# ActiveIntelligentSystemsLab/moving_object_detector

Hardware: AMD Instinct MI355X
Metric: stereo pairs/sec (scene-flow+cluster) at 1280x720 (higher is better)
Workload: dtype f32+f64; 1 GPU; 1280x720 synthetic sequence (zed-style camera), scene-flow + cluster kernels only (disparity/flow precomputed, HBM-resident), reference default parameters; distinct_frames_per_gpu=16, outputs=six cloud planes, dynamic mask, objects, cluster-label plane, batch_chunks=0, stream=one synthetic stream, contiguous chunk per rank + one disparity plane of halo, collective_executed=True, collective_backend=nccl, collective_on_device=True, collective_world_size=1

## Files before the change

moving_object_detector_amd/csrc/cluster_final.hip:

```cpp
#include "cluster_common.h"
#include <algorithm>
#pragma clang fp contract(off)
namespace {

#ifndef FINAL_PLAIN_LABELS
#define FINAL_ST(p, v) __builtin_nontemporal_store((int)(v), (p))
#else
#define FINAL_ST(p, v) (*(p) = (v))
#endif
constexpr int kFinalEarly = 32;
template <int TH, int NW, bool XY_FROM_Z>
__global__ __launch_bounds__(NW * 64) void k_final(DevCam c, ClArgs a) {
  constexpr int RPW = TH / NW;
  __shared__ int nlmap[TH * 64];
  __shared__ int lcount[TH * 64];
  const int wi = blockIdx.x, f = blockIdx.z, lane = threadIdx.x, w = __builtin_amdgcn_readfirstlane((int)threadIdx.y);
  const size_t tidx = (size_t)f * gridDim.y * gridDim.x + (size_t)blockIdx.y * gridDim.x + wi;
  const size_t N = (size_t)c.W * c.H;
  const size_t fN = (size_t)f * N;
  const int x0 = wi * 64, y0 = blockIdx.y * TH, r0 = w * RPW, x = x0 + lane;
  if (a.tilehdr[tidx * 2] == 0) {
    if (a.labels) {
#pragma unroll
      for (int j = 0; j < RPW; j++) { const int y = y0 + r0 + j; if (y < c.H && x < c.W) FINAL_ST(&a.labels[fN + (size_t)y * c.W + x], -1); }
    }
    return;
  }
  const int xc = min(x, c.W - 1);
  uint64_t mw[RPW], rw[RPW];
  int par[RPW];
#pragma unroll
  for (int j = 0; j < RPW; j++) {
    const int y = y0 + r0 + j, yc = min(y, c.H - 1);
    const size_t wo = ((size_t)f * c.H + yc) * c.mask_words + wi;
    mw[j] = (y < c.H) ? a.mask[wo] : 0ull;
    rw[j] = (y < c.H) ? a.lroot[wo] : 0ull;
    par[j] = a.parent[fN + (size_t)yc * c.W + xc];
  }
#pragma unroll
  for (int j = 0; j < RPW; j++) {
    if ((rw[j] >> lane) & 1ull) {
      const int cell = (r0 + j) * 64 + lane;
      const int p = (y0 + r0 + j) * c.W + x;
      int lab = -1, first = 0;
      if (MOD_CHECK(a, par[j] >= 0 && (size_t)par[j] < N, 5)) {
        const int fr = par[j];
        lab = a.rkey[fN + fr];
        const int seg = a.rsize[fN + fr];
        const int own = a.rkey[fN + p];
        first = seg + (fr == p ? 0 : own);
      }
      nlmap[cell] = lab;
      lcount[cell] = first;
    }
  }
  float vx[RPW], vy[RPW], vz[RPW], px[RPW], py[RPW], pz[RPW];
  int ndyn = 0;
#pragma unroll
  for (int j = 0; j < RPW; j++) ndyn += __popcll((unsigned long long)mw[j]);
  const bool early = ndyn >= kFinalEarly;
  auto load_members = [&]() {
#pragma unroll
    for (int j = 0; j < RPW; j++) {
      const size_t gp = fN + (size_t)min(y0 + r0 + j, c.H - 1) * c.W + xc;
      vx[j] = a.vx[gp]; vy[j] = a.vy[gp]; vz[j] = a.vz[gp];
      pz[j] = a.z[gp];
      if (!XY_FROM_Z) { px[j] = a.x[gp]; py[j] = a.y[gp]; }
    }
  };
  if (early) load_members();
  lds_barrier();
  if (w == 0 && lane == 0) a.tilehdr[tidx * 2] = 0;
  const float invW = 1.0f / (float)c.W;
  const int tile0 = y0 * c.W + x0;
  int nl[RPW], cell[RPW], slot[RPW];
  bool any_member = false;
#pragma unroll
  for (int j = 0; j < RPW; j++) {
    const int y = y0 + r0 + j;
    const bool dyn = (mw[j] >> lane) & 1ull;
    const int d = par[j] - tile0;
    const int ly = (int)(((float)d + 0.5f) * invW);
    const bool isroot = (rw[j] >> lane) & 1ull;
    int cl = !dyn ? 0 : isroot ? ((r0 + j) * 64 + lane) : (ly * 64 + (d - ly * c.W));
    if (!MOD_CHECK(a, cl >= 0 && cl < TH * 64 && (!dyn || isroot || (d >= 0 && d - ly * c.W < 64)), 6)) cl = 0;
    int l = dyn ? nlmap[cl] : -1;
    if (!MOD_CHECK(a, l >= -1 && l < a.max_objects, 7)) l = -1;
    nl[j] = l; cell[j] = cl; slot[j] = 0;
    if (a.labels && y < c.H && x < c.W) FINAL_ST(&a.labels[fN + (size_t)y * c.W + x], l);
    any_member = any_member || (__ballot(l >= 0) != 0);
  }
  if (any_member) {
    if (!early) load_members();
#pragma unroll
    for (int j = 0; j < RPW; j++) {
      const int l = nl[j], cl = cell[j];
      const uint64_t mb = __ballot(l >= 0);
      if (mb == 0) continue;
      const int lead = __ffsll((unsigned long long)mb) - 1;
      const int c0 = __builtin_amdgcn_readlane(cl, lead);
      const bool grp = l >= 0 && cl == c0;
      const uint64_t gb = __ballot(grp);
      int base = 0;
      if (lane == lead) base = atomicAdd(&lcount[c0], __popcll((unsigned long long)gb));
      base = __builtin_amdgcn_readlane(base, lead);
      if (grp) slot[j] = base + __popcll((unsigned long long)(gb & ((1ull << lane) - 1ull)));
      else if (l >= 0) slot[j] = atomicAdd(&lcount[cl], 1);
    }
    if (XY_FROM_Z) {
      const double rx = c.rayx[xc];
#pragma unroll
      for (int j = 0; j < RPW; j++) {
        const double zd = (double)pz[j];
        px[j] = (float)(rx * zd);
        py[j] = (float)(c.rayy[min(y0 + r0 + j, c.H - 1)] * zd);
      }
    }
    uint32_t nb[RPW];
#pragma unroll
    for (int j = 0; j < RPW; j++) nb[j] = __float_as_uint(norm3_f32(vx[j], vy[j], vz[j]));
#pragma unroll
    for (int j = 0; j < RPW; j++) {
      if (nl[j] >= 0) {
        if (MOD_CHECK(a, slot[j] >= 0 && (size_t)slot[j] < N, 8)) {
          a.mbits[fN + slot[j]] = nb[j];
          a.mpix[fN + slot[j]] = (uint32_t)((y0 + r0 + j) * c.W + x);
        }
      }
    }
    int pend[RPW];
#pragma unroll
    for (int j = 0; j < RPW; j++) pend[j] = nl[j];
    for (;;) {
      int mine = -1;
#pragma unroll
      for (int j = 0; j < RPW; j++) mine = pend[j] >= 0 ? pend[j] : mine;
      const uint64_t b = __ballot(mine >= 0);
      if (b == 0) break;
      const int L = __builtin_amdgcn_readlane(mine, __ffsll((unsigned long long)b) - 1);
      uint32_t mn0 = 0xffffffffu, mn1 = 0xffffffffu, mn2 = 0xffffffffu, mx0 = 0u, mx1 = 0u, mx2 = 0u, mn3 = 0xffffffffu, mx3 = 0u;
#pragma unroll
      for (int j = 0; j < RPW; j++) {
        if (pend[j] == L) {
          const uint32_t ox = f2ord(px[j]), oy = f2ord(py[j]), oz = f2ord(pz[j]);
          mn0 = min(mn0, ox); mx0 = max(mx0, ox); mn1 = min(mn1, oy); mx1 = max(mx1, oy); mn2 = min(mn2, oz); mx2 = max(mx2, oz);
          mn3 = min(mn3, nb[j]); mx3 = max(mx3, nb[j]);
          pend[j] = -1;
        }
      }
      mn0 = wave_min_u32(mn0); mn1 = wave_min_u32(mn1); mn2 = wave_min_u32(mn2); mn3 = wave_min_u32(mn3);
      mx0 = wave_max_u32(mx0); mx1 = wave_max_u32(mx1); mx2 = wave_max_u32(mx2); mx3 = wave_max_u32(mx3);
      uint32_t v = ~mx3;
      v = lane == 0 ? mn0 : v; v = lane == 1 ? mn1 : v; v = lane == 2 ? mn2 : v; v = lane == 3 ? ~mx0 : v; v = lane == 4 ? ~mx1 : v;
// ... 44 lines not shown
  uint32_t *cstart = reinterpret_cast<uint32_t *>(&lraw[kMemCells]);
  __shared__ int s_box[4], s_sum[kMemThreads / 64 + 1];
  for (int f = blockIdx.x; f < frames; f += gridDim.x) {
    const ClusterInfo *C = a.clusters + (size_t)f * a.max_objects;
    const int K = min(a.counters[f * kClusterCounters + 1], a.max_objects);
    const int total = K > 0 ? C[K - 1].offset + C[K - 1].size : 0;
    int32_t *o = m.offsets + (size_t)f * (a.max_objects + 1);
    for (int k = tid; k <= a.max_objects; k += kMemThreads) o[k] = k < K ? C[k].offset : total;
  }
  auto segment = [&](uint32_t item, int &size, int &off) {
    const ClusterInfo *ci = a.clusters + item;
    size = ci->size; off = ci->offset;
    return size >= 1 && off >= 0 && (size_t)off + (size_t)size <= N;
  };
  for (int wi = blockIdx.x; wi < nwork; wi += gridDim.x) {
    const uint32_t item = a.worklist[wi];
    int size, off;
    if (!segment(item, size, off) || size <= kMemWaveMax) continue;
    members_of<kMemThreads, kMemCells, XY_FROM_Z, POINTS>(c, a, m, item, size, off, cmask, cstart, s_box, s_sum, tid);
  }
  __syncthreads();
  for (int wi = blockIdx.x * (kMemThreads / 64) + wv; wi < nwork; wi += gridDim.x * (kMemThreads / 64)) {
    const uint32_t item = a.worklist[wi];
    int size, off;
    if (!segment(item, size, off) || size > kMemWaveMax) continue;
    members_of<64, kMemWaveCells, XY_FROM_Z, POINTS>(c, a, m, item, size, off, cmask + wv * kMemWaveCells, cstart + wv * kMemWaveCells, nullptr,
                                                     nullptr, lane);
  }
}
}

void launch_final(const DevCam &c, const ClArgs &a, int frames, hipStream_t s) {
  constexpr int kFinalWaves = 2;
  if (a.xy_from_z) hipLaunchKernelGGL((k_final<kTileH, kFinalWaves, true>), tile_grid(c, frames), dim3(64, kFinalWaves, 1), 0, s, c, a);
  else hipLaunchKernelGGL((k_final<kTileH, kFinalWaves, false>), tile_grid(c, frames), dim3(64, kFinalWaves, 1), 0, s, c, a);
}

void launch_cluster_members(const DevCam &c, const ClArgs &a, const ClusterMemberOut &m, int frames, hipStream_t s) {
  const dim3 grid(std::min(256, frames * 4)), block(kMemThreads);
  const bool pts = m.points != nullptr;
  if (a.xy_from_z) {
    if (pts) hipLaunchKernelGGL((k_cluster_members<true, true>), grid, block, 0, s, c, a, m, frames);
    else hipLaunchKernelGGL((k_cluster_members<true, false>), grid, block, 0, s, c, a, m, frames);
  } else {
    if (pts) hipLaunchKernelGGL((k_cluster_members<false, true>), grid, block, 0, s, c, a, m, frames);
    else hipLaunchKernelGGL((k_cluster_members<false, false>), grid, block, 0, s, c, a, m, frames);
  }
}
```

moving_object_detector_amd/csrc/mod_context.h:

```cpp
#pragma once
#include "../../include/mod_sf.h"
#include "frame_const.h"
#include "mod_launch.h"

#include <string>
#include <utility>
#include <vector>

constexpr int kRing = 4;
constexpr int kMaxChunks = 4;

template <class H, auto Release>
class Owned {
  H h_ = nullptr;

 public:
  Owned() = default;
  Owned(Owned &&o) noexcept : h_(std::exchange(o.h_, nullptr)) {}
  Owned &operator=(Owned &&o) noexcept { std::swap(h_, o.h_); return *this; }
  ~Owned() { reset(); }
  operator H() const { return h_; }
  H get() const { return h_; }
  H *put() { reset(); return &h_; }
  void reset() { if (h_) (void)Release(h_); h_ = nullptr; }
};
template <class T> using DevPtr = Owned<T *, hipFree>;
template <class T> using HostPtr = Owned<T *, hipHostFree>;
using Event = Owned<hipEvent_t, hipEventDestroy>;
using Stream = Owned<hipStream_t, hipStreamDestroy>;

template <class T>
hipError_t dalloc(DevPtr<T> &p, size_t count) { return p ? hipSuccess : hipMalloc((void **)p.put(), count * sizeof(T)); }
inline hipError_t make_event(Event &e) { return e ? hipSuccess : hipEventCreateWithFlags(e.put(), hipEventDisableTiming); }
#define HIP_OK(expr) do { if (hipError_t e_ = (expr); e_ != hipSuccess) return e_; } while (0)

struct Fence {
  Event ev;
  bool armed = false;
  hipError_t record(hipStream_t s) {
    hipError_t e = make_event(ev);
    if (e == hipSuccess && (e = hipEventRecord(ev, s)) == hipSuccess) armed = true;
    return e;
  }
  hipError_t wait(hipStream_t s) const { return armed ? hipStreamWaitEvent(s, ev, 0) : hipSuccess; }
  hipError_t wait_once(hipStream_t s) { return std::exchange(armed, false) ? hipStreamWaitEvent(s, ev, 0) : hipSuccess; }
};

struct EventPair { Event a, b; };

struct ClusterScratch {
  size_t frames = 0, pixels = 0, mask_rows = 0, tiles = 0, max_objects = 0;
  DevPtr<uint64_t> mask, lroot;
  DevPtr<float2> zrange;
  DevPtr<int32_t> parent, rsize, rkey;
  DevPtr<uint32_t> mbits, mpix;
  DevPtr<ClusterBox> cbox;
  DevPtr<ClusterInfo> clusters;
  DevPtr<uint32_t> worklist;
  ClusterInfo *rank_scratch = nullptr; uint32_t *tielist = nullptr;
  DevPtr<int32_t> counters, tilehdr;
  DevPtr<uint32_t> tilelist;
  DevPtr<uint2> requests; size_t req_alloc = 0;
};

struct Buffers {
  DevPtr<double> rayx, rayy;
  DevPtr<FrameConst> fc;
  DevPtr<unsigned long long> dbg;
  ClusterScratch cluster;
  struct Sgm {
    DevPtr<uint32_t> census;
    DevPtr<uint8_t> maps;
    DevPtr<uint8_t> S;
    int D = 0, G = 0; bool maps16 = false;
    Stream side[kSgmPaths];
    Event fork[2], join[2][kSgmPaths];
  } sgm;
  struct Speckle { DevPtr<int32_t> parent, size; int frames = 0; } spk;
  struct Flow {
    DevPtr<uint8_t> img;
    DevPtr<uint32_t> census;
    DevPtr<short2> winners;
    DevPtr<short4> sub;
  } flow;
  struct Ego {
    DevPtr<double> corr, hyp;
    DevPtr<uint8_t> flag; size_t cap = 0;
    DevPtr<int32_t> blkcnt, ncorr, hcnt;
// ... 183 lines not shown
```

moving_object_detector_amd/csrc/mod_launch.h:

```cpp
#pragma once
#include "../../include/mod_sf.h"
#include "mod_device.h"

struct SfArgs {
  const float *dnow, *dprev, *flow;
  float *x, *y, *z, *vx, *vy, *vz;
  uint64_t *mask;
  float4 *aos;
  float *depth;
  float *sflow;
  const FrameConst *fc;
  int32_t *tilehdr;
  int32_t tile_rows, tiles_x, tiles_per_frame;
  float2 *zrange;
  unsigned long long *dbg;
};

constexpr int kClusterCounters = 8;
constexpr int kTileHdrWords = 2;

struct ClArgs {
  const float *x, *y, *z, *vx, *vy, *vz;
  const uint64_t *mask;
  const float2 *zrange;
  uint64_t *lroot;
  int32_t *parent;
  int32_t *rootlist;
  int32_t *labels;
  int32_t *rsize;
  int32_t *rkey;
  ClusterBox *cbox;
  int32_t *counters;
  ClusterInfo *clusters;
  uint32_t *mbits;
  uint32_t *mpix;
  uint32_t *worklist;
  uint32_t *tielist;
  void *objects;
  int32_t *n_objects;
  int32_t *n_clusters;
  int32_t max_objects;
  int32_t xy_from_z;
  uint2 *requests;
  int32_t *tilehdr;
  uint32_t *tilelist;
  int32_t req_cap;
  unsigned long long *dbg;
};

#define MOD_SF_INLINE_FRAMES 8
void launch_scene_flow(const DevCam &c, const SfArgs &a, int frames, const FrameConst *inline_consts, hipStream_t s);
void launch_dynamic_mask(const DevCam &c, int frames, const float *vx, const float *vy, const float *vz, uint64_t *mask,
                         hipStream_t s);
void launch_depth(const DevCam &c, int frames, const float *dnow, float *depth, hipStream_t s);
void launch_copy_words(const unsigned long long *src, unsigned long long *dst, size_t n, hipStream_t s);
void launch_pack(size_t n, const float *x, const float *y, const float *z, const float *vx, const float *vy, const float *vz,
                 void *aos, hipStream_t s);
// ... 91 lines not shown
```

moving_object_detector_amd/csrc/mod_sf.hip:

```cpp
#include "mod_context.h"
#include "exact_div.h"
#include "mod_sf_debug.h"

#include <algorithm>
#include <cmath>
#include <cstdlib>
#include <limits>

namespace {

constexpr int kChunkMinFrames = 32;
constexpr int kAutoChunks = 1;

float ceil_to_f32(double th) {
  if (std::isnan(th)) return std::nanf("");
  float t = (float)th;
  if ((double)t < th) t = std::nextafterf(t, INFINITY);
  return t;
}
float floor_to_f32(double th) {
  if (std::isnan(th)) return std::nanf("");
  float t = (float)th;
  if ((double)t > th) t = std::nextafterf(t, -INFINITY);
  return t;
// ... 49 lines not shown
    return MOD_OK;
  }
  const int slot = c->ring_pos;
  c->ring_pos = (c->ring_pos + 1) % kRing;
  HIP_TRY(c, hipEventSynchronize(c->pinned_ev[slot]));
  FrameConst *h = c->pinned[slot];
  for (int f = 0; f < in->frames; f++) fill_frame_const(h[f], in->transforms[f], in->dt[f]);
  launch_copy_words((const unsigned long long *)h, (unsigned long long *)c->b.fc.get(), sizeof(FrameConst) / 8 * (size_t)in->frames, c->stream);
  HIP_TRY(c, hipGetLastError());
  HIP_TRY(c, hipEventRecord(c->pinned_ev[slot], c->stream));
  return MOD_OK;
}

int check_batch(ModContext *c, const ModFrameBatch *in) {
  if (!in) return fail(c, MOD_ERR_INVALID_ARGUMENT, "null batch");
  int rc = check_ready(c, in->frames);
  if (rc) return rc;
  return construct_skip(in->flow, in->disparity_prev, in->transforms && in->dt, in->disparity_now);
}

struct Chunk { int f0, n; };

template <class T> T *at(T *p, size_t f0, size_t stride) { return p ? p + f0 * stride : nullptr; }

hipError_t cluster_alloc(ClusterScratch &s, const ModConfig &cfg, int max_objects) {
  s.frames = (size_t)cfg.max_frames; s.pixels = (size_t)cfg.max_width * cfg.max_height; s.max_objects = (size_t)max_objects;
  s.mask_rows = (size_t)mod_mask_words(cfg.max_width) * cfg.max_height; s.tiles = (size_t)ccl_tiles(mod_mask_words(cfg.max_width), cfg.max_height);
  const size_t F = s.frames, FN = F * s.pixels, FM = F * s.mask_rows, FO = F * s.max_objects, FT = F * s.tiles;
  HIP_OK(dalloc(s.mask, FM)); HIP_OK(dalloc(s.lroot, FM)); HIP_OK(dalloc(s.zrange, FM));
  HIP_OK(dalloc(s.parent, FN)); HIP_OK(dalloc(s.rsize, FN)); HIP_OK(dalloc(s.rkey, FN));
  HIP_OK(dalloc(s.cbox, FO)); HIP_OK(dalloc(s.counters, F * kClusterCounters));
  HIP_OK(dalloc(s.clusters, 2 * FO)); s.rank_scratch = s.clusters + FO;
  HIP_OK(dalloc(s.mbits, FN)); HIP_OK(dalloc(s.mpix, FN));
  HIP_OK(dalloc(s.worklist, 2 * FO)); s.tielist = s.worklist + FO;
  HIP_OK(dalloc(s.tilehdr, FT * kTileHdrWords));
  return dalloc(s.tilelist, FT);
}

hipError_t cluster_grow_requests(ClusterScratch &s, int n, hipStream_t stream) {
  const size_t need = s.frames * s.tiles * ccl_request_capacity(n);
  if (need <= s.req_alloc) return hipSuccess;
  HIP_OK(hipStreamSynchronize(stream));
  s.requests.reset(); s.req_alloc = 0;
  HIP_OK(dalloc(s.requests, need));
  s.req_alloc = need; return hipSuccess;
}

struct Carved { ClArgs a; ClusterInfo *rank_scratch; float2 *zrange; int tiles; ClusterMemberOut members; };

Carved cluster_carve(const Buffers &b, const DevCam &dc, Chunk ch, const ModSceneFlowPlanes *pl, const uint64_t *mask, bool flags_ready, const ModClusterOut *out,
                     const ModClusterMembers *mem) {
  const ClusterScratch &s = b.cluster;
  const size_t N = (size_t)dc.W * dc.H, f0 = (size_t)ch.f0, MWH = (size_t)dc.mask_words * dc.H, MO = s.max_objects, tiles = (size_t)ccl_tiles(dc.mask_words, dc.H);
  static const ModClusterOut no_out{}; if (!out) out = &no_out;
  Carved v{{}, s.rank_scratch + f0 * MO, s.zrange + f0 * MWH, (int)tiles, {}}; ClArgs &a = v.a;
  if (mem) v.members = {at(mem->offsets, f0, MO + 1), at(mem->indices, f0, N), at(mem->points, f0, 3 * N)};
  a.x = at(pl->x, f0, N); a.y = at(pl->y, f0, N); a.z = at(pl->z, f0, N); a.vx = at(pl->vx, f0, N); a.vy = at(pl->vy, f0, N); a.vz = at(pl->vz, f0, N);
  a.mask = at(mask, f0, MWH); a.zrange = flags_ready ? v.zrange : nullptr; a.lroot = s.lroot + f0 * MWH;
  a.parent = s.parent + f0 * N; a.rootlist = (int32_t *)s.mpix.get() + f0 * N; a.rsize = s.rsize + f0 * N; a.rkey = s.rkey + f0 * N;
  a.cbox = s.cbox + f0 * MO; a.counters = s.counters + f0 * kClusterCounters; a.clusters = s.clusters + f0 * MO;
  a.mbits = s.mbits + f0 * N; a.mpix = s.mpix + f0 * N; a.worklist = s.worklist + f0 * MO; a.tielist = s.tielist + f0 * MO;
  a.labels = at(out->labels, f0, N); a.objects = at(out->objects, f0, MO); a.n_objects = at(out->n_objects, f0, 1); a.n_clusters = at(out->n_clusters, f0, 1);
  a.max_objects = (int32_t)MO; a.req_cap = ccl_request_capacity(dc.n); a.dbg = b.dbg; a.xy_from_z = flags_ready ? 1 : 0;
  a.requests = s.requests + f0 * tiles * (size_t)a.req_cap; a.tilehdr = s.tilehdr + f0 * tiles * kTileHdrWords; a.tilelist = s.tilelist + f0 * tiles;
  return v;
}

int check_scene_flow_out(ModContext *c, const ModSceneFlowPlanes *out, bool xy_optional) {
  if (!out || !out->z || !out->vx || !out->vy || !out->vz)
    return fail(c, MOD_ERR_INVALID_ARGUMENT, "scene-flow output planes z,vx,vy,vz are required");
  if ((out->x == nullptr) != (out->y == nullptr) || (!out->x && !xy_optional))
    return fail(c, MOD_ERR_INVALID_ARGUMENT, xy_optional ? "scene-flow output planes x and y: pass both or neither" : "scene-flow output planes x,y,z,vx,vy,vz are required");
  return MOD_OK;
}

void enqueue_scene_flow(ModContext *c, const ModFrameBatch *in, const ModSceneFlowPlanes *out, uint64_t *mask, bool tile_flags, Chunk ch,
                        hipStream_t s, const InlineConsts *inl = nullptr) {
  const size_t N = (size_t)c->dc.W * c->dc.H, f0 = (size_t)ch.f0;
  const bool marks = tile_flags && mask;
  const Carved cv = cluster_carve(c->b, c->dc, ch, out, mask, marks, nullptr, nullptr);
  SfArgs a;
  a.dnow = in->disparity_now + f0 * N; a.dprev = in->disparity_prev + f0 * N; a.flow = in->flow + f0 * N * 2;
  a.x = at(out->x, f0, N); a.y = at(out->y, f0, N); a.z = out->z + f0 * N; a.vx = out->vx + f0 * N; a.vy = out->vy + f0 * N; a.vz = out->vz + f0 * N;
  a.mask = at(mask, f0, (size_t)c->dc.mask_words * c->dc.H);
  a.aos = at((float4 *)out->cloud_aos, f0, N * 2); a.depth = at(out->depth, f0, N); a.sflow = at(out->static_flow, f0, N * 2);
  a.fc = c->b.fc + f0; a.dbg = c->b.dbg;
  a.tilehdr = marks ? cv.a.tilehdr : nullptr;
  a.zrange = marks ? cv.zrange : nullptr;
  a.tile_rows = ccl_tile_rows(); a.tiles_x = c->dc.mask_words; a.tiles_per_frame = cv.tiles;
  StageTimer t(c, MOD_STAGE_SCENE_FLOW, s);
  launch_scene_flow(c->dc, a, ch.n, (inl && inl->used) ? inl->v : nullptr, s);
}

int run_scene_flow(ModContext *c, const ModFrameBatch *in, const ModSceneFlowPlanes *out, uint64_t *mask, bool tile_flags, bool xy_optional) {
  int rc = check_scene_flow_out(c, out, xy_optional);
  if (rc) return rc;
  InlineConsts inl;
  if ((rc = upload_frame_consts(c, in, &inl))) return rc;
  enqueue_scene_flow(c, in, out, mask, tile_flags, Chunk{0, in->frames}, c->stream, &inl);
  HIP_TRY(c, hipGetLastError());
  return MOD_OK;
}

int check_cluster_io(ModContext *c, const ModSceneFlowPlanes *pl, bool flags_ready, const ModClusterOut *out) {
  if (!pl || !pl->z || !pl->vx || !pl->vy || !pl->vz || (!flags_ready && (!pl->x || !pl->y)))
    return fail(c, MOD_ERR_INVALID_ARGUMENT, "cluster input planes x,y,z,vx,vy,vz are required");
  if (!out || !out->objects || !out->n_objects)
    return fail(c, MOD_ERR_INVALID_ARGUMENT, "cluster outputs objects, n_objects are required");
  return MOD_OK;
}

void enqueue_cluster(ModContext *c, Chunk ch, const ModSceneFlowPlanes *pl, const uint64_t *mask, bool mask_ready, bool flags_ready,
                    const ModClusterOut *out, const ModClusterMembers *mem, hipStream_t s) {
  const Carved cv = cluster_carve(c->b, c->dc, ch, pl, mask, flags_ready, out, mem);
  const ClArgs &a = cv.a;
  const int frames = ch.n;
  {
    StageTimer t(c, MOD_STAGE_CCL_TILE, s);
    if (!mask_ready) launch_dynamic_mask(c->dc, frames, a.vx, a.vy, a.vz, (uint64_t *)a.mask, s);
    if (!flags_ready) launch_tile_flags(c->dc, a, frames, s);
    launch_ccl_tile(c->dc, a, frames, s);
// ... 382 lines not shown
```

moving_object_detector_amd/csrc/sceneflow.hip:

```cpp
#include <cstddef>
#include <type_traits>

#include "exact_div.h"
#include "mod_launch.h"
#include <algorithm>

#pragma clang fp contract(off)

namespace {

struct Px {
  float x, y, z, vx, vy, vz, s0, s1, depth;
  bool dyn;
};

__device__ __forceinline__ bool disp_in_range(const DevCam &c, float d) {
  return !(c.dmax < d) && !(c.dmin > d);
}

__device__ __forceinline__ void iso_apply(const FrameConst &fc, float X, float Y, float Z, float &ox, float &oy, float &oz) {
  const double x = (double)X, y = (double)Y, z = (double)Z;
  ox = (float)(fc.m[3] + (fc.m[0] * x + (fc.m[1] * y + fc.m[2] * z)));
  oy = (float)(fc.m[7] + (fc.m[4] * x + (fc.m[5] * y + fc.m[6] * z)));
  oz = (float)(fc.m[11] + (fc.m[8] * x + (fc.m[9] * y + fc.m[10] * z)));
// ... 106 lines not shown
__device__ __forceinline__ uint64_t nibbles_to_word(uint32_t nib, int lane) {
  uint32_t v = nib << (4 * (lane & 7));
  v |= MOD_DPP(v, 0xB1);
  v |= MOD_DPP(v, 0x4E);
  v |= MOD_DPP(v, 0x141);
  const uint32_t hi = MOD_DPP(v, 0x108);
  return (uint64_t)v | ((uint64_t)hi << 32);
}

__device__ __forceinline__ float sf_min(float a, float b) { float r; asm("v_min_f32 %0, %1, %2" : "=v"(r) : "v"(a), "v"(b)); return r; }
__device__ __forceinline__ float sf_max(float a, float b) { float r; asm("v_max_f32 %0, %1, %2" : "=v"(r) : "v"(a), "v"(b)); return r; }
#define SF_DPPF(v, ctrl) __uint_as_float(MOD_DPP(__float_as_uint(v), ctrl))
__device__ __forceinline__ void row16_minmax(float &mn, float &mx) {
  mn = sf_min(mn, SF_DPPF(mn, 0xB1)); mx = sf_max(mx, SF_DPPF(mx, 0xB1));
  mn = sf_min(mn, SF_DPPF(mn, 0x4E)); mx = sf_max(mx, SF_DPPF(mx, 0x4E));
  mn = sf_min(mn, SF_DPPF(mn, 0x141)); mx = sf_max(mx, SF_DPPF(mx, 0x141));
  mn = sf_min(mn, SF_DPPF(mn, 0x140)); mx = sf_max(mx, SF_DPPF(mx, 0x140));
}
template <int G> __device__ __forceinline__ void group_minmax(float &mn, float &mx) {
#pragma unroll
  for (int o = 1; o < G; o <<= 1) { mn = sf_min(mn, __shfl_xor(mn, o)); mx = sf_max(mx, __shfl_xor(mx, o)); }
}

template <class T> __device__ __forceinline__ T ld(const void *base, uint32_t byte_off) {
  return *reinterpret_cast<const T *>(reinterpret_cast<const char *>(base) + byte_off);
}
template <class T> __device__ __forceinline__ void st(void *base, uint32_t byte_off, const T &v) {
  *reinterpret_cast<T *>(reinterpret_cast<char *>(base) + byte_off) = v;
}
__device__ __forceinline__ void st_plane(float *base, uint32_t byte_off, float a0, float a1, float a2, float a3) {
  typedef float sf_w4 __attribute__((ext_vector_type(4)));
  const sf_w4 v = {a0, a1, a2, a3};
  asm volatile("global_store_dwordx4 %0, %1, %2 sc0 sc1 nt" :: "v"(byte_off), "v"(v), "s"(base) : "memory");
}
#define SF_K4 __attribute__((address_space(4)))
template <class T> __device__ __forceinline__ T karg(size_t off) {
  const SF_K4 char *kp = (const SF_K4 char *)__builtin_amdgcn_kernarg_segment_ptr();
  return *(const volatile SF_K4 T *)(kp + off);
}
constexpr size_t kSfArgsAt = (sizeof(DevCam) + alignof(SfArgs) - 1) / alignof(SfArgs) * alignof(SfArgs);
#define LATE_A(field) karg<decltype(SfArgs::field)>(kSfArgsAt + offsetof(SfArgs, field))
struct SfKernargLayout { DevCam c; SfArgs a; };
static_assert(std::is_trivially_copyable<DevCam>::value && std::is_trivially_copyable<SfArgs>::value, "kernarg structs are copied bytewise");
static_assert(alignof(DevCam) <= 8 && alignof(SfArgs) <= 8, "kernarg segment is 8-byte aligned per argument here");
static_assert(kSfArgsAt == offsetof(SfKernargLayout, a), "SfArgs does not sit where karg() reads it");
constexpr int kSfInlineFrames = MOD_SF_INLINE_FRAMES;
struct SfConsts { FrameConst v[kSfInlineFrames]; };
struct SfKernargLayoutInl { DevCam c; SfArgs a; SfConsts k; };
static_assert(std::is_trivially_copyable<SfConsts>::value && alignof(SfConsts) <= 8, "kernarg struct");
template <bool INL> __device__ __forceinline__ FrameConst frame_const(const SfArgs &a, int f) {
  if (INL) {
    const SF_K4 char *kp = (const SF_K4 char *)__builtin_amdgcn_kernarg_segment_ptr();
    const SF_K4 double *q = (const SF_K4 double *)(kp + offsetof(SfKernargLayoutInl, k) + (size_t)f * sizeof(FrameConst));
    static_assert(sizeof(FrameConst) == 16 * sizeof(double), "FrameConst is 16 doubles");
    FrameConst r;
#pragma unroll
    for (int i = 0; i < 12; i++) r.m[i] = q[i];
    r.dt = q[12]; r.pad[0] = q[13]; r.pad[1] = q[14]; r.pad[2] = q[15];
    return r;
  }
  return a.fc[f];
}

template <bool XY, bool INL>
__device__ __forceinline__ void sf_v4_body(const DevCam &c, const SfArgs &a) {
  const int lane = threadIdx.x;
  uint32_t bx = blockIdx.x, by = blockIdx.y, bz = blockIdx.z;
  {
    const uint32_t rows = gridDim.y * gridDim.z;
    if ((rows & 7u) == 0u && !MOD_ABLATE(c, 64)) {
      const uint32_t lin = bx + gridDim.x * (by + gridDim.y * bz);
      const uint32_t j = lin >> 3, k = lin & 7u;
      const uint32_t r = j / gridDim.x * 8u + k;
      bx = j % gridDim.x;
      by = r % gridDim.y; bz = r / gridDim.y;
    }
  }
  const int x0 = (bx * 64 + lane) * 4;
  const int y = by * 4 + threadIdx.y;
  const int f = bz;
  const bool inb = (x0 < c.W) && (y < c.H);
  const size_t fN = (size_t)f * ((size_t)c.W * c.H);
  const uint32_t pix = (uint32_t)y * (uint32_t)c.W + (uint32_t)x0;
  const uint32_t o4 = pix * 4u, o8 = pix * 8u;
  const FrameConst fc = frame_const<INL>(a, f);
  uint32_t nib = 0;
  uint64_t *out_mask = nullptr;
  int32_t *out_hdr = nullptr;
  float2 *out_zr = nullptr;
  const float qnan = __uint_as_float(0x7fc00000u);
  float zmn = qnan, zmx = qnan;
  if (inb) {
    const float *dprev_f = a.dprev + fN;
    const float4 dn = ld<float4>(a.dnow + fN, o4);
    const float4 dp = ld<float4>(dprev_f, o4);
    const float4 fa = ld<float4>(a.flow + 2 * fN, o8);
    const float4 fb = ld<float4>(a.flow + 2 * fN, o8 + 16u);
    const double ry = c.rayy[y];
    const double2 rxa = ld<double2>(c.rayx, (uint32_t)x0 * 8u);
    const double2 rxb = ld<double2>(c.rayx, (uint32_t)x0 * 8u + 16u);
    Px p0, p1, p2, p3;
    PxState s0, s1, s2, s3;
    sf_stage1(c, fc, x0 + 0, y, dn.x, dp.x, fa.x, fa.y, rxa.x, ry, p0, s0);
    sf_stage1(c, fc, x0 + 1, y, dn.y, dp.y, fa.z, fa.w, rxa.y, ry, p1, s1);
    sf_stage1(c, fc, x0 + 2, y, dn.z, dp.z, fb.x, fb.y, rxb.x, ry, p2, s2);
    sf_stage1(c, fc, x0 + 3, y, dn.w, dp.w, fb.z, fb.w, rxb.y, ry, p3, s3);
    if (XY) {
      st_plane(a.x + fN, o4, p0.x, p1.x, p2.x, p3.x);
      st_plane(a.y + fN, o4, p0.y, p1.y, p2.y, p3.y);
    }
    st_plane(a.z + fN, o4, p0.z, p1.z, p2.z, p3.z);
    float *const out_vx = LATE_A(vx), *const out_vy = LATE_A(vy), *const out_vz = LATE_A(vz);
#ifdef MOD_CHECKED
    if (out_vx != a.vx || LATE_A(tilehdr) != a.tilehdr || LATE_A(tiles_x) != a.tiles_x) {
      if (a.dbg) atomicAdd(&a.dbg[kDbgCheckBase + 16], 1ull);
      return;
    }
#endif
    float4 *const out_aos = LATE_A(aos);
    float *const out_depth = LATE_A(depth), *const out_sflow = LATE_A(sflow);
    out_mask = LATE_A(mask); out_hdr = LATE_A(tilehdr); out_zr = LATE_A(zrange);
    const uint32_t W = (uint32_t)c.W;
    const float g0 = ld<float>(dprev_f, ((uint32_t)s0.py * W + (uint32_t)s0.px) * 4u);
    const float g1 = ld<float>(dprev_f, ((uint32_t)s1.py * W + (uint32_t)s1.px) * 4u);
    const float g2 = ld<float>(dprev_f, ((uint32_t)s2.py * W + (uint32_t)s2.px) * 4u);
    const float g3 = ld<float>(dprev_f, ((uint32_t)s3.py * W + (uint32_t)s3.px) * 4u);
    const double ax0 = ld<double>(c.rayx, (uint32_t)s0.px * 8u), ax1 = ld<double>(c.rayx, (uint32_t)s1.px * 8u);
    const double ax2 = ld<double>(c.rayx, (uint32_t)s2.px * 8u), ax3 = ld<double>(c.rayx, (uint32_t)s3.px * 8u);
    const double ay0 = ld<double>(c.rayy, (uint32_t)s0.py * 8u), ay1 = ld<double>(c.rayy, (uint32_t)s1.py * 8u);
    const double ay2 = ld<double>(c.rayy, (uint32_t)s2.py * 8u), ay3 = ld<double>(c.rayy, (uint32_t)s3.py * 8u);
    PxWarp w0, w1, w2, w3;
    sf_stage2a(c, fc, s0, g0, ax0, ay0, p0, w0);
    sf_stage2a(c, fc, s1, g1, ax1, ay1, p1, w1);
    sf_stage2a(c, fc, s2, g2, ax2, ay2, p2, w2);
    sf_stage2a(c, fc, s3, g3, ax3, ay3, p3, w3);
    if (__any(w0.todo | w1.todo | w2.todo | w3.todo)) {
      sf_stage2b(c, fc, s0, w0, p0);
      sf_stage2b(c, fc, s1, w1, p1);
      sf_stage2b(c, fc, s2, w2, p2);
      sf_stage2b(c, fc, s3, w3, p3);
    }
    st_plane(out_vx + fN, o4, p0.vx, p1.vx, p2.vx, p3.vx);
    st_plane(out_vy + fN, o4, p0.vy, p1.vy, p2.vy, p3.vy);
    st_plane(out_vz + fN, o4, p0.vz, p1.vz, p2.vz, p3.vz);
    if (out_aos) {
      float4 *q = out_aos + 2 * fN;
      const uint32_t o32 = pix * 32u;
      st(q, o32, make_float4(p0.x, p0.y, p0.z, 0.f)); st(q, o32 + 16u, make_float4(p0.vx, p0.vy, p0.vz, 0.f));
      st(q, o32 + 32u, make_float4(p1.x, p1.y, p1.z, 0.f)); st(q, o32 + 48u, make_float4(p1.vx, p1.vy, p1.vz, 0.f));
      st(q, o32 + 64u, make_float4(p2.x, p2.y, p2.z, 0.f)); st(q, o32 + 80u, make_float4(p2.vx, p2.vy, p2.vz, 0.f));
      st(q, o32 + 96u, make_float4(p3.x, p3.y, p3.z, 0.f)); st(q, o32 + 112u, make_float4(p3.vx, p3.vy, p3.vz, 0.f));
    }
    if (out_depth) st(out_depth + fN, o4, make_float4(p0.depth, p1.depth, p2.depth, p3.depth));
    if (out_sflow) {
      st(out_sflow + 2 * fN, o8, make_float4(p0.s0, p0.s1, p1.s0, p1.s1));
      st(out_sflow + 2 * fN, o8 + 16u, make_float4(p2.s0, p2.s1, p3.s0, p3.s1));
    }
    nib = (p0.dyn ? 1u : 0u) | (p1.dyn ? 2u : 0u) | (p2.dyn ? 4u : 0u) | (p3.dyn ? 8u : 0u);
    if (__any(nib != 0u)) {
      const float z0 = p0.dyn ? s0.zn : qnan, z1 = p1.dyn ? s1.zn : qnan, z2 = p2.dyn ? s2.zn : qnan, z3 = p3.dyn ? s3.zn : qnan;
      zmn = sf_min(sf_min(z0, z1), sf_min(z2, z3)); zmx = sf_max(sf_max(z0, z1), sf_max(z2, z3));
    }
  }
  if (!inb) { out_mask = LATE_A(mask); out_hdr = LATE_A(tilehdr); out_zr = LATE_A(zrange); }
  if (out_mask) {
    const uint64_t w = nibbles_to_word(nib, lane);
    const int word = (bx * 64 + lane) / 16;
    if (out_zr && __any(nib != 0u)) row16_minmax(zmn, zmx);
    if ((lane & 15) == 0 && y < c.H && word < c.mask_words) {
      const size_t wo = ((size_t)f * c.H + y) * c.mask_words + word;
      out_mask[wo] = w;
      if (out_hdr && w) out_hdr[((size_t)f * LATE_A(tiles_per_frame) + (size_t)(y / LATE_A(tile_rows)) * LATE_A(tiles_x) + word) * 2] = 1;
      if (out_zr && w) out_zr[wo] = make_float2(zmn, zmx);
    }
  }
}


template <bool XY> __global__ __launch_bounds__(256) void k_scene_flow_v4(DevCam c, SfArgs a) { sf_v4_body<XY, false>(c, a); }
template <bool XY> __global__ __launch_bounds__(256) void k_scene_flow_v4i(DevCam c, SfArgs a, SfConsts k) { sf_v4_body<XY, true>(c, a); }

template <bool INL>
__device__ __forceinline__ void sf_v2_body(const DevCam &c, const SfArgs &a) {
  const int lane = threadIdx.x;
  const int x0 = (blockIdx.x * 64 + lane) * 2;
  const int y = blockIdx.y * 4 + threadIdx.y;
  const int f = blockIdx.z;
  const bool inb = (x0 < c.W) && (y < c.H);
  const size_t fN = (size_t)f * ((size_t)c.W * c.H);
  const uint32_t pix = (uint32_t)y * (uint32_t)c.W + (uint32_t)x0;
  const uint32_t o4 = pix * 4u, o8 = pix * 8u;
  const FrameConst fc = frame_const<INL>(a, f);
  uint32_t two = 0;
  const float qnan = __uint_as_float(0x7fc00000u);
  float zmn = qnan, zmx = qnan;
  if (inb) {
    const float *dprev_f = a.dprev + fN;
    const float2 dn = ld<float2>(a.dnow + fN, o4);
    const float2 dp = ld<float2>(dprev_f, o4);
    const float4 fl = ld<float4>(a.flow + 2 * fN, o8);
    const double ry = c.rayy[y];
    const double2 rx = ld<double2>(c.rayx, (uint32_t)x0 * 8u);
    Px p0, p1;
    PxState s0, s1;
    sf_stage1(c, fc, x0 + 0, y, dn.x, dp.x, fl.x, fl.y, rx.x, ry, p0, s0);
    sf_stage1(c, fc, x0 + 1, y, dn.y, dp.y, fl.z, fl.w, rx.y, ry, p1, s1);
    if (a.x) {
      st(a.x + fN, o4, make_float2(p0.x, p1.x));
      st(a.y + fN, o4, make_float2(p0.y, p1.y));
    }
    st(a.z + fN, o4, make_float2(p0.z, p1.z));
    const uint32_t W = (uint32_t)c.W;
    const float g0 = ld<float>(dprev_f, ((uint32_t)s0.py * W + (uint32_t)s0.px) * 4u);
    const float g1 = ld<float>(dprev_f, ((uint32_t)s1.py * W + (uint32_t)s1.px) * 4u);
    const double ax0 = ld<double>(c.rayx, (uint32_t)s0.px * 8u), ax1 = ld<double>(c.rayx, (uint32_t)s1.px * 8u);
    const double ay0 = ld<double>(c.rayy, (uint32_t)s0.py * 8u), ay1 = ld<double>(c.rayy, (uint32_t)s1.py * 8u);
    PxWarp w0, w1;
    sf_stage2a(c, fc, s0, g0, ax0, ay0, p0, w0);
    sf_stage2a(c, fc, s1, g1, ax1, ay1, p1, w1);
    if (__any(w0.todo | w1.todo)) {
      sf_stage2b(c, fc, s0, w0, p0);
      sf_stage2b(c, fc, s1, w1, p1);
    }
    st(a.vx + fN, o4, make_float2(p0.vx, p1.vx));
    st(a.vy + fN, o4, make_float2(p0.vy, p1.vy));
    st(a.vz + fN, o4, make_float2(p0.vz, p1.vz));
    if (a.aos) {
      float4 *q = a.aos + 2 * fN;
      const uint32_t o32 = pix * 32u;
      st(q, o32, make_float4(p0.x, p0.y, p0.z, 0.f)); st(q, o32 + 16u, make_float4(p0.vx, p0.vy, p0.vz, 0.f));
      st(q, o32 + 32u, make_float4(p1.x, p1.y, p1.z, 0.f)); st(q, o32 + 48u, make_float4(p1.vx, p1.vy, p1.vz, 0.f));
    }
    if (a.depth) st(a.depth + fN, o4, make_float2(p0.depth, p1.depth));
    if (a.sflow) st(a.sflow + 2 * fN, o8, make_float4(p0.s0, p0.s1, p1.s0, p1.s1));
    two = (p0.dyn ? 1u : 0u) | (p1.dyn ? 2u : 0u);
    zmn = sf_min(p0.dyn ? p0.z : qnan, p1.dyn ? p1.z : qnan); zmx = sf_max(p0.dyn ? p0.z : qnan, p1.dyn ? p1.z : qnan);
  }
  if (a.mask) {
    uint32_t v = two << (2 * (lane & 15));
    v |= __shfl_xor(v, 1); v |= __shfl_xor(v, 2); v |= __shfl_xor(v, 4); v |= __shfl_xor(v, 8);
    const uint32_t hi = __shfl_down(v, 16);
    const int word = blockIdx.x * 2 + (lane >> 5);
    if (a.zrange) group_minmax<32>(zmn, zmx);
    if ((lane & 31) == 0 && y < c.H && word < c.mask_words) {
      const uint64_t wd = (uint64_t)v | ((uint64_t)hi << 32);
      const size_t wo = ((size_t)f * c.H + y) * c.mask_words + word;
      a.mask[wo] = wd;
      if (a.tilehdr && wd) a.tilehdr[((size_t)f * a.tiles_per_frame + (size_t)(y / a.tile_rows) * a.tiles_x + word) * 2] = 1;
      if (a.zrange && wd) a.zrange[wo] = make_float2(zmn, zmx);
    }
  }
}

__global__ __launch_bounds__(256) void k_scene_flow_v2(DevCam c, SfArgs a) { sf_v2_body<false>(c, a); }
__global__ __launch_bounds__(256) void k_scene_flow_v2i(DevCam c, SfArgs a, SfConsts k) { sf_v2_body<true>(c, a); }

template <bool INL>
__device__ __forceinline__ void sf_v1_body(const DevCam &c, const SfArgs &a) {
  const int lane = threadIdx.x;
  const int x = blockIdx.x * 64 + lane;
  const int y = blockIdx.y * 4 + threadIdx.y;
  const int f = blockIdx.z;
  const bool inb = (x < c.W) && (y < c.H);
  const size_t N = (size_t)c.W * c.H;
  const size_t i = (size_t)f * N + (size_t)y * c.W + x;
  const FrameConst fc = frame_const<INL>(a, f);
  bool dyn = false;
  const float qnan = __uint_as_float(0x7fc00000u);
  float zmn = qnan, zmx = qnan;
  if (inb) {
    Px p;
    sf_pixel(c, fc, a.dprev + (size_t)f * N, x, y, a.dnow[i], a.dprev[i], a.flow[2 * i], a.flow[2 * i + 1], c.rayx[x], c.rayy[y], p);
    if (a.x) { a.x[i] = p.x; a.y[i] = p.y; }
    a.z[i] = p.z; a.vx[i] = p.vx; a.vy[i] = p.vy; a.vz[i] = p.vz;
    if (a.aos) { a.aos[2 * i] = make_float4(p.x, p.y, p.z, 0.f); a.aos[2 * i + 1] = make_float4(p.vx, p.vy, p.vz, 0.f); }
    if (a.depth) a.depth[i] = p.depth;
    if (a.sflow) { a.sflow[2 * i] = p.s0; a.sflow[2 * i + 1] = p.s1; }
    dyn = p.dyn;
    zmn = zmx = dyn ? p.z : qnan;
  }
  if (a.mask) {
    const uint64_t w = __ballot(dyn);
    if (a.zrange) group_minmax<64>(zmn, zmx);
    if (lane == 0 && y < c.H && blockIdx.x < (unsigned)c.mask_words) {
      const size_t wo = ((size_t)f * c.H + y) * c.mask_words + blockIdx.x;
      a.mask[wo] = w;
      if (a.tilehdr && w) a.tilehdr[((size_t)f * a.tiles_per_frame + (size_t)(y / a.tile_rows) * a.tiles_x + blockIdx.x) * 2] = 1;
      if (a.zrange && w) a.zrange[wo] = make_float2(zmn, zmx);
    }
  }
}
__global__ __launch_bounds__(256) void k_scene_flow_v1(DevCam c, SfArgs a) { sf_v1_body<false>(c, a); }
__global__ __launch_bounds__(256) void k_scene_flow_v1i(DevCam c, SfArgs a, SfConsts k) { sf_v1_body<true>(c, a); }

__global__ __launch_bounds__(256) void k_dynamic_mask(DevCam c, const float *__restrict__ vx, const float *__restrict__ vy,
                                                      const float *__restrict__ vz, uint64_t *__restrict__ mask) {
  const int lane = threadIdx.x;
  const int x = blockIdx.x * 64 + lane;
  const int y = blockIdx.y * 4 + threadIdx.y;
  const int f = blockIdx.z;
  bool dyn = false;
  if (x < c.W && y < c.H) {
    const size_t i = ((size_t)f * c.H + y) * c.W + x;
    dyn = sumsq3_f32(vx[i], vy[i], vz[i]) >= c.speed_th_sq;
  }
  const uint64_t w = __ballot(dyn);
  if (lane == 0 && y < c.H && blockIdx.x < (unsigned)c.mask_words) mask[((size_t)f * c.H + y) * c.mask_words + blockIdx.x] = w;
}

__global__ __launch_bounds__(256) void k_depth(DevCam c, size_t n, const float *__restrict__ dnow, float *__restrict__ depth) {
  const size_t i = (size_t)blockIdx.x * 256 + threadIdx.x;
  if (i >= n) return;
  const float d = dnow[i];
  const bool ok = disp_in_range(c, d) & !(d == 0.0f);
  depth[i] = ok ? c.fT / d : __uint_as_float(0x7fc00000u);
}
// ... 66 lines not shown
```

Before: 100,700 stereo pairs/s.

## Precompute velocity norms in scene-flow and read a norm plane in final

The scene-flow kernels now compute the velocity magnitude for pixels in dynamic groups and write it to a new scratch norm plane. The final cluster kernel then loads one float per pixel instead of three velocity components and skips loads for rows with no dynamic pixels. This cuts read traffic and recomputation in k_final, at the cost of an extra strided store in the scene-flow pass plus one more scratch allocation. A fenced store variant with an s_nop is also added.

```diff
diff --git a/moving_object_detector_amd/csrc/cluster_final.hip b/moving_object_detector_amd/csrc/cluster_final.hip
--- a/moving_object_detector_amd/csrc/cluster_final.hip
+++ b/moving_object_detector_amd/csrc/cluster_final.hip
@@ -9,7 +9,7 @@
 #define FINAL_ST(p, v) (*(p) = (v))
 #endif
 constexpr int kFinalEarly = 32;
-template <int TH, int NW, bool XY_FROM_Z>
+template <int TH, int NW, bool XY_FROM_Z, bool NORMS>
 __global__ __launch_bounds__(NW * 64) void k_final(DevCam c, ClArgs a) {
   constexpr int RPW = TH / NW;
   __shared__ int nlmap[TH * 64];
@@ -62,8 +62,11 @@
   auto load_members = [&]() {
 #pragma unroll
     for (int j = 0; j < RPW; j++) {
+      vx[j] = vy[j] = vz[j] = px[j] = py[j] = pz[j] = 0.0f;
+      if (__builtin_amdgcn_readfirstlane((int)((uint32_t)mw[j] | (uint32_t)(mw[j] >> 32))) == 0) continue;
       const size_t gp = fN + (size_t)min(y0 + r0 + j, c.H - 1) * c.W + xc;
-      vx[j] = a.vx[gp]; vy[j] = a.vy[gp]; vz[j] = a.vz[gp];
+      if (NORMS) vx[j] = a.vnorm[gp];
+      else { vx[j] = a.vx[gp]; vy[j] = a.vy[gp]; vz[j] = a.vz[gp]; }
       pz[j] = a.z[gp];
       if (!XY_FROM_Z) { px[j] = a.x[gp]; py[j] = a.y[gp]; }
     }
@@ -118,7 +121,7 @@
     }
     uint32_t nb[RPW];
 #pragma unroll
-    for (int j = 0; j < RPW; j++) nb[j] = __float_as_uint(norm3_f32(vx[j], vy[j], vz[j]));
+    for (int j = 0; j < RPW; j++) nb[j] = NORMS ? __float_as_uint(vx[j]) : __float_as_uint(norm3_f32(vx[j], vy[j], vz[j]));
 #pragma unroll
     for (int j = 0; j < RPW; j++) {
       if (nl[j] >= 0) {
@@ -229,8 +232,9 @@
 
 void launch_final(const DevCam &c, const ClArgs &a, int frames, hipStream_t s) {
   constexpr int kFinalWaves = 2;
-  if (a.xy_from_z) hipLaunchKernelGGL((k_final<kTileH, kFinalWaves, true>), tile_grid(c, frames), dim3(64, kFinalWaves, 1), 0, s, c, a);
-  else hipLaunchKernelGGL((k_final<kTileH, kFinalWaves, false>), tile_grid(c, frames), dim3(64, kFinalWaves, 1), 0, s, c, a);
+  if (a.xy_from_z && a.vnorm) hipLaunchKernelGGL((k_final<kTileH, kFinalWaves, true, true>), tile_grid(c, frames), dim3(64, kFinalWaves, 1), 0, s, c, a);
+  else if (a.xy_from_z) hipLaunchKernelGGL((k_final<kTileH, kFinalWaves, true, false>), tile_grid(c, frames), dim3(64, kFinalWaves, 1), 0, s, c, a);
+  else hipLaunchKernelGGL((k_final<kTileH, kFinalWaves, false, false>), tile_grid(c, frames), dim3(64, kFinalWaves, 1), 0, s, c, a);
 }
 
 void launch_cluster_members(const DevCam &c, const ClArgs &a, const ClusterMemberOut &m, int frames, hipStream_t s) {
diff --git a/moving_object_detector_amd/csrc/mod_context.h b/moving_object_detector_amd/csrc/mod_context.h
--- a/moving_object_detector_amd/csrc/mod_context.h
+++ b/moving_object_detector_amd/csrc/mod_context.h
@@ -54,6 +54,7 @@
   DevPtr<float2> zrange;
   DevPtr<int32_t> parent, rsize, rkey;
   DevPtr<uint32_t> mbits, mpix;
+  DevPtr<float> vnorm;
   DevPtr<ClusterBox> cbox;
   DevPtr<ClusterInfo> clusters;
   DevPtr<uint32_t> worklist;
diff --git a/moving_object_detector_amd/csrc/mod_launch.h b/moving_object_detector_amd/csrc/mod_launch.h
--- a/moving_object_detector_amd/csrc/mod_launch.h
+++ b/moving_object_detector_amd/csrc/mod_launch.h
@@ -14,7 +14,14 @@
   int32_t tile_rows, tiles_x, tiles_per_frame;
   float2 *zrange;
   unsigned long long *dbg;
+  float *vnorm;
 };
+
+#ifdef FINAL_NORMS_FROM_VELOCITY
+constexpr bool kFinalNormPlane = false;
+#else
+constexpr bool kFinalNormPlane = true;
+#endif
 
 constexpr int kClusterCounters = 8;
 constexpr int kTileHdrWords = 2;
@@ -23,6 +30,7 @@
   const float *x, *y, *z, *vx, *vy, *vz;
   const uint64_t *mask;
   const float2 *zrange;
+  const float *vnorm;
   uint64_t *lroot;
   int32_t *parent;
   int32_t *rootlist;
diff --git a/moving_object_detector_amd/csrc/mod_sf.hip b/moving_object_detector_amd/csrc/mod_sf.hip
--- a/moving_object_detector_amd/csrc/mod_sf.hip
+++ b/moving_object_detector_amd/csrc/mod_sf.hip
@@ -105,6 +105,7 @@
   HIP_OK(dalloc(s.cbox, FO)); HIP_OK(dalloc(s.counters, F * kClusterCounters));
   HIP_OK(dalloc(s.clusters, 2 * FO)); s.rank_scratch = s.clusters + FO;
   HIP_OK(dalloc(s.mbits, FN)); HIP_OK(dalloc(s.mpix, FN));
+  if (kFinalNormPlane) HIP_OK(dalloc(s.vnorm, FN));
   HIP_OK(dalloc(s.worklist, 2 * FO)); s.tielist = s.worklist + FO;
   HIP_OK(dalloc(s.tilehdr, FT * kTileHdrWords));
   return dalloc(s.tilelist, FT);
@@ -119,17 +120,17 @@
   s.req_alloc = need; return hipSuccess;
 }
 
-struct Carved { ClArgs a; ClusterInfo *rank_scratch; float2 *zrange; int tiles; ClusterMemberOut members; };
+struct Carved { ClArgs a; ClusterInfo *rank_scratch; float2 *zrange; float *vnorm; int tiles; ClusterMemberOut members; };
 
 Carved cluster_carve(const Buffers &b, const DevCam &dc, Chunk ch, const ModSceneFlowPlanes *pl, const uint64_t *mask, bool flags_ready, const ModClusterOut *out,
                      const ModClusterMembers *mem) {
   const ClusterScratch &s = b.cluster;
   const size_t N = (size_t)dc.W * dc.H, f0 = (size_t)ch.f0, MWH = (size_t)dc.mask_words * dc.H, MO = s.max_objects, tiles = (size_t)ccl_tiles(dc.mask_words, dc.H);
   static const ModClusterOut no_out{}; if (!out) out = &no_out;
-  Carved v{{}, s.rank_scratch + f0 * MO, s.zrange + f0 * MWH, (int)tiles, {}}; ClArgs &a = v.a;
+  Carved v{{}, s.rank_scratch + f0 * MO, s.zrange + f0 * MWH, at(s.vnorm.get(), f0, N), (int)tiles, {}}; ClArgs &a = v.a;
   if (mem) v.members = {at(mem->offsets, f0, MO + 1), at(mem->indices, f0, N), at(mem->points, f0, 3 * N)};
   a.x = at(pl->x, f0, N); a.y = at(pl->y, f0, N); a.z = at(pl->z, f0, N); a.vx = at(pl->vx, f0, N); a.vy = at(pl->vy, f0, N); a.vz = at(pl->vz, f0, N);
-  a.mask = at(mask, f0, MWH); a.zrange = flags_ready ? v.zrange : nullptr; a.lroot = s.lroot + f0 * MWH;
+  a.mask = at(mask, f0, MWH); a.zrange = flags_ready ? v.zrange : nullptr; a.vnorm = flags_ready ? v.vnorm : nullptr; a.lroot = s.lroot + f0 * MWH;
   a.parent = s.parent + f0 * N; a.rootlist = (int32_t *)s.mpix.get() + f0 * N; a.rsize = s.rsize + f0 * N; a.rkey = s.rkey + f0 * N;
   a.cbox = s.cbox + f0 * MO; a.counters = s.counters + f0 * kClusterCounters; a.clusters = s.clusters + f0 * MO;
   a.mbits = s.mbits + f0 * N; a.mpix = s.mpix + f0 * N; a.worklist = s.worklist + f0 * MO; a.tielist = s.tielist + f0 * MO;
@@ -160,6 +161,7 @@
   a.fc = c->b.fc + f0; a.dbg = c->b.dbg;
   a.tilehdr = marks ? cv.a.tilehdr : nullptr;
   a.zrange = marks ? cv.zrange : nullptr;
+  a.vnorm = marks ? cv.vnorm : nullptr;
   a.tile_rows = ccl_tile_rows(); a.tiles_x = c->dc.mask_words; a.tiles_per_frame = cv.tiles;
   StageTimer t(c, MOD_STAGE_SCENE_FLOW, s);
   launch_scene_flow(c->dc, a, ch.n, (inl && inl->used) ? inl->v : nullptr, s);
diff --git a/moving_object_detector_amd/csrc/sceneflow.hip b/moving_object_detector_amd/csrc/sceneflow.hip
--- a/moving_object_detector_amd/csrc/sceneflow.hip
+++ b/moving_object_detector_amd/csrc/sceneflow.hip
@@ -162,6 +162,11 @@
   typedef float sf_w4 __attribute__((ext_vector_type(4)));
   const sf_w4 v = {a0, a1, a2, a3};
   asm volatile("global_store_dwordx4 %0, %1, %2 sc0 sc1 nt" :: "v"(byte_off), "v"(v), "s"(base) : "memory");
+}
+__device__ __forceinline__ void st_plane_fenced(float *base, uint32_t byte_off, float a0, float a1, float a2, float a3) {
+  typedef float sf_w4 __attribute__((ext_vector_type(4)));
+  const sf_w4 v = {a0, a1, a2, a3};
+  asm volatile("global_store_dwordx4 %0, %1, %2 sc0 sc1 nt\n\ts_nop 1" :: "v"(byte_off), "v"(v), "s"(base) : "memory");
 }
 #define SF_K4 __attribute__((address_space(4)))
 template <class T> __device__ __forceinline__ T karg(size_t off) {
@@ -220,6 +225,9 @@
   float2 *out_zr = nullptr;
   const float qnan = __uint_as_float(0x7fc00000u);
   float zmn = qnan, zmx = qnan;
+#ifndef FINAL_NORMS_FROM_VELOCITY
+  float n0 = 0.0f, n1 = 0.0f, n2 = 0.0f, n3 = 0.0f;
+#endif
   if (inb) {
     const float *dprev_f = a.dprev + fN;
     const float4 dn = ld<float4>(a.dnow + fN, o4);
@@ -250,6 +258,9 @@
     float4 *const out_aos = LATE_A(aos);
     float *const out_depth = LATE_A(depth), *const out_sflow = LATE_A(sflow);
     out_mask = LATE_A(mask); out_hdr = LATE_A(tilehdr); out_zr = LATE_A(zrange);
+#ifndef FINAL_NORMS_FROM_VELOCITY
+    float *const out_vn = LATE_A(vnorm);
+#endif
     const uint32_t W = (uint32_t)c.W;
     const float g0 = ld<float>(dprev_f, ((uint32_t)s0.py * W + (uint32_t)s0.px) * 4u);
     const float g1 = ld<float>(dprev_f, ((uint32_t)s1.py * W + (uint32_t)s1.px) * 4u);
@@ -290,13 +301,29 @@
     if (__any(nib != 0u)) {
       const float z0 = p0.dyn ? s0.zn : qnan, z1 = p1.dyn ? s1.zn : qnan, z2 = p2.dyn ? s2.zn : qnan, z3 = p3.dyn ? s3.zn : qnan;
       zmn = sf_min(sf_min(z0, z1), sf_min(z2, z3)); zmx = sf_max(sf_max(z0, z1), sf_max(z2, z3));
+#ifndef FINAL_NORMS_FROM_VELOCITY
+      if (out_vn) {
+        n0 = norm3_f32(p0.vx, p0.vy, p0.vz); n1 = norm3_f32(p1.vx, p1.vy, p1.vz);
+        n2 = norm3_f32(p2.vx, p2.vy, p2.vz); n3 = norm3_f32(p3.vx, p3.vy, p3.vz);
+      }
+#endif
     }
   }
   if (!inb) { out_mask = LATE_A(mask); out_hdr = LATE_A(tilehdr); out_zr = LATE_A(zrange); }
   if (out_mask) {
+#ifndef FINAL_NORMS_FROM_VELOCITY
+    float *const out_vn = LATE_A(vnorm);
+#endif
     const uint64_t w = nibbles_to_word(nib, lane);
     const int word = (bx * 64 + lane) / 16;
     if (out_zr && __any(nib != 0u)) row16_minmax(zmn, zmx);
+#ifndef FINAL_NORMS_FROM_VELOCITY
+    if (out_vn && __any(nib != 0u)) {
+      const uint32_t half = (uint32_t)w;
+      const uint32_t both = half | MOD_DPP(half, 0x140);
+      if (inb && both != 0u) st_plane_fenced(out_vn + fN, o4, n0, n1, n2, n3);
+    }
+#endif
     if ((lane & 15) == 0 && y < c.H && word < c.mask_words) {
       const size_t wo = ((size_t)f * c.H + y) * c.mask_words + word;
       out_mask[wo] = w;
@@ -324,6 +351,9 @@
   uint32_t two = 0;
   const float qnan = __uint_as_float(0x7fc00000u);
   float zmn = qnan, zmx = qnan;
+#ifndef FINAL_NORMS_FROM_VELOCITY
+  float n0 = 0.0f, n1 = 0.0f;
+#endif
   if (inb) {
     const float *dprev_f = a.dprev + fN;
     const float2 dn = ld<float2>(a.dnow + fN, o4);
@@ -364,6 +394,9 @@
     if (a.depth) st(a.depth + fN, o4, make_float2(p0.depth, p1.depth));
     if (a.sflow) st(a.sflow + 2 * fN, o8, make_float4(p0.s0, p0.s1, p1.s0, p1.s1));
     two = (p0.dyn ? 1u : 0u) | (p1.dyn ? 2u : 0u);
+#ifndef FINAL_NORMS_FROM_VELOCITY
+    if (a.vnorm) { n0 = norm3_f32(p0.vx, p0.vy, p0.vz); n1 = norm3_f32(p1.vx, p1.vy, p1.vz); }
+#endif
     zmn = sf_min(p0.dyn ? p0.z : qnan, p1.dyn ? p1.z : qnan); zmx = sf_max(p0.dyn ? p0.z : qnan, p1.dyn ? p1.z : qnan);
   }
   if (a.mask) {
@@ -372,6 +405,12 @@
     const uint32_t hi = __shfl_down(v, 16);
     const int word = blockIdx.x * 2 + (lane >> 5);
     if (a.zrange) group_minmax<32>(zmn, zmx);
+#ifndef FINAL_NORMS_FROM_VELOCITY
+    if (a.vnorm) {
+      const uint32_t both = v | __shfl_xor(v, 16);
+      if (inb && both != 0u) st(a.vnorm + fN, o4, make_float2(n0, n1));
+    }
+#endif
     if ((lane & 31) == 0 && y < c.H && word < c.mask_words) {
       const uint64_t wd = (uint64_t)v | ((uint64_t)hi << 32);
       const size_t wo = ((size_t)f * c.H + y) * c.mask_words + word;
@@ -398,6 +437,9 @@
   bool dyn = false;
   const float qnan = __uint_as_float(0x7fc00000u);
   float zmn = qnan, zmx = qnan;
+#ifndef FINAL_NORMS_FROM_VELOCITY
+  float vn = 0.0f;
+#endif
   if (inb) {
     Px p;
     sf_pixel(c, fc, a.dprev + (size_t)f * N, x, y, a.dnow[i], a.dprev[i], a.flow[2 * i], a.flow[2 * i + 1], c.rayx[x], c.rayy[y], p);
@@ -408,10 +450,16 @@
     if (a.sflow) { a.sflow[2 * i] = p.s0; a.sflow[2 * i + 1] = p.s1; }
     dyn = p.dyn;
     zmn = zmx = dyn ? p.z : qnan;
+#ifndef FINAL_NORMS_FROM_VELOCITY
+    if (a.vnorm) vn = norm3_f32(p.vx, p.vy, p.vz);
+#endif
   }
   if (a.mask) {
     const uint64_t w = __ballot(dyn);
     if (a.zrange) group_minmax<64>(zmn, zmx);
+#ifndef FINAL_NORMS_FROM_VELOCITY
+    if (a.vnorm && w && inb) a.vnorm[i] = vn;
+#endif
     if (lane == 0 && y < c.H && blockIdx.x < (unsigned)c.mask_words) {
       const size_t wo = ((size_t)f * c.H + y) * c.mask_words + blockIdx.x;
       a.mask[wo] = w;
```

Result: no change. 100,700 stereo pairs/s (-0.0%).
